# nquach/TEE_optical_flow

Measured on AMD Instinct MI355X. Metric: frame-pairs/sec @512x512 DualTVL1, higher is better.
Workload: dtype f32

## Files before the change

tee_optical_flow_amd/csrc/teeflow_dbg.hip.h:

```cpp
namespace {
template <class T> struct DevBuf { T* p = nullptr; ~DevBuf() { if (p) (void)hipFree(p); } };
using DBuf = DevBuf<float>;

int dbg_up(tf_handle* h, DBuf& d, const float* src, const Geom& g)
{
    HIPC(h, hipMalloc(&d.p, (size_t)g.plane * sizeof(float)));
    HIPC(h, hipMemsetAsync(d.p, 0, (size_t)g.plane * sizeof(float), h->stream));
    if (src) HIPC(h, hipMemcpy2DAsync(d.p, (size_t)g.pitch * 4, src, (size_t)g.w * 4, (size_t)g.w * 4, g.h, hipMemcpyHostToDevice, h->stream));
    return TF_OK;
}
int dbg_down(tf_handle* h, float* dst, const float* d, const Geom& g)
{
    HIPC(h, hipMemcpy2DAsync(dst, (size_t)g.w * 4, d, (size_t)g.pitch * 4, (size_t)g.w * 4, g.h, hipMemcpyDeviceToHost, h->stream));
    HIPC(h, hipStreamSynchronize(h->stream));
    return TF_OK;
}

int dbg_up2(tf_handle* h, DBuf& fr, const float* I0, const float* I1, const Geom& g)
{
    HIPC(h, hipMalloc(&fr.p, 2 * (size_t)g.plane * sizeof(float)));
    HIPC(h, hipMemsetAsync(fr.p, 0, 2 * (size_t)g.plane * sizeof(float), h->stream));
    HIPC(h, hipMemcpy2DAsync(fr.p, (size_t)g.pitch * 4, I0, (size_t)g.w * 4, (size_t)g.w * 4, g.h, hipMemcpyHostToDevice, h->stream));
    HIPC(h, hipMemcpy2DAsync(fr.p + g.plane, (size_t)g.pitch * 4, I1, (size_t)g.w * 4, (size_t)g.w * 4, g.h, hipMemcpyHostToDevice, h->stream));
    return TF_OK;
// ... 204 lines not shown
    const Geom g = make_geom(w, hgt);
    DBuf a0, a1, b0, b1;
    int rc;
    if ((rc = dbg_up(h, a0, src, g)) || (rc = dbg_up(h, a1, nullptr, g)) || (rc = dbg_up(h, b0, src, g)) || (rc = dbg_up(h, b1, nullptr, g))) return rc;
    DevBuf<PairCtl> ctl;
    HIPC(h, hipMalloc(&ctl.p, sizeof(PairCtl)));
    HIPC(h, hipMemsetAsync(ctl.p, 0, sizeof(PairCtl), h->stream));
    MedArgs ma = {};
    ma.sb.u1[0] = a0.p; ma.sb.u1[1] = a1.p; ma.sb.u2[0] = b0.p; ma.sb.u2[1] = b1.p;
    ma.ctl = ctl.p; ma.err = nullptr; ma.errstride = 0; ma.it = 0; ma.thr_q = 0; ma.utog = 0; ma.g = g;
    ma.total = 1; ma.step = iter_step(h, false, h->P.inner_iterations);
    const dim3 gm((g.w + 63) / 64, (g.h + 15) / 16, 2);
    if (ksize == 5) hipLaunchKernelGGL(k_median<5>, gm, dim3(256), 0, h->stream, ma);
    else hipLaunchKernelGGL(k_median<3>, gm, dim3(256), 0, h->stream, ma);
    hipError_t e = hipStreamSynchronize(h->stream);
    if (e != hipSuccess) return fail(h, TF_ERR_HIP, "k_median: %s", hipGetErrorString(e));
    return dbg_down(h, dst, a1.p, g);
}

TF_API int tf_dbg_iterate(tf_handle* h, const float* I1wx, const float* I1wy, const float* rho_c,
                          float* u1, float* u2, float* p11, float* p12, float* p21, float* p22,
                          int w, int hgt, int nsteps, int p_is_zero, unsigned long long* err_q)
{
    if (!h || !I1wx || !I1wy || !rho_c || !u1 || !u2 || !p11 || !p12 || !p21 || !p22 || w < 1 || hgt < 1 || nsteps < 0)
        return TF_ERR_INVALID_ARG;
    HIPC(h, hipSetDevice(h->dev));
    const Geom g = make_geom(w, hgt);
    DBuf cx, cy, cr, s[12];
    int rc;
    if ((rc = dbg_up(h, cx, I1wx, g)) || (rc = dbg_up(h, cy, I1wy, g)) || (rc = dbg_up(h, cr, rho_c, g))) return rc;
    float* hostp[6] = {u1, u2, p11, p12, p21, p22};
    for (int k = 0; k < 6; ++k) {
        if ((rc = dbg_up(h, s[2 * k], hostp[k], g)) || (rc = dbg_up(h, s[2 * k + 1], nullptr, g))) return rc;
    }
    DevBuf<PairCtl> ctl; DevBuf<u64> errs;
    HIPC(h, hipMalloc(&ctl.p, sizeof(PairCtl)));
    HIPC(h, hipMemsetAsync(ctl.p, 0, sizeof(PairCtl), h->stream));
    HIPC(h, hipMalloc(&errs.p, (size_t)(nsteps + 1) * sizeof(u64)));
    HIPC(h, hipMemsetAsync(errs.p, 0, (size_t)(nsteps + 1) * sizeof(u64), h->stream));
    Iter2Args A = {};
    IterArgs& ia = A.a;
    ia.wx = cx.p; ia.wy = cy.p; ia.rho = cr.p;
    for (int k = 0; k < 2; ++k) {
        ia.sb.u1[k] = s[0 + k].p; ia.sb.u2[k] = s[2 + k].p; ia.sb.p11[k] = s[4 + k].p;
        ia.sb.p12[k] = s[6 + k].p; ia.sb.p21[k] = s[8 + k].p; ia.sb.p22[k] = s[10 + k].p;
    }
    ia.ctl = ctl.p; ia.err = errs.p; ia.errstride = nsteps + 1; ia.thr_q = -1.0; ia.g = g; ia.host_slot = nullptr; ia.B = 1;
    ia.l_t = (float)(h->P.lambda * h->P.theta); ia.theta = (float)h->P.theta; ia.taut = (float)(h->P.tau / h->P.theta);
    const int step = iter_step(h, false, nsteps);
    A.total = nsteps;
    int launches = 0;
    for (int it = 0; it < nsteps; it += step, ++launches) {
        ia.it = it; ia.utog = ia.ptog = launches; ia.pzero = (p_is_zero && it == 0) ? 1 : 0;
        launch_iter(h, A, step, 1, h->stream);
    }
    hipError_t e = hipStreamSynchronize(h->stream);
    if (e == hipSuccess && err_q && nsteps > 0) {
        e = hipMemcpyAsync(err_q, errs.p, (size_t)nsteps * sizeof(u64), hipMemcpyDeviceToHost, h->stream);
        if (e == hipSuccess) e = hipStreamSynchronize(h->stream);
    }
    if (e != hipSuccess) return fail(h, TF_ERR_HIP, "k_iter: %s", hipGetErrorString(e));
    const int cur = launches & 1;
    for (int k = 0; k < 6; ++k)
        if ((rc = dbg_down(h, hostp[k], s[2 * k + cur].p, g))) return rc;
    return TF_OK;
}
```

tee_optical_flow_amd/csrc/teeflow_tvl1_host.hip.h:

```cpp
namespace {
int validate_params(Engine* h, const tf_params& p)
{
    if (p.algo != TF_ALGO_TVL1) return fail(h, TF_ERR_UNSUPPORTED, "algo %d not implemented (only TF_ALGO_TVL1)", p.algo);
    if (p.nscales < 1 || p.nscales > MAXLEV) return fail(h, TF_ERR_INVALID_ARG, "nscales must be in [1,%d], got %d", MAXLEV, p.nscales);
    if (p.warps < 1) return fail(h, TF_ERR_INVALID_ARG, "warps must be >= 1, got %d", p.warps);
    if (p.inner_iterations < 1 || p.outer_iterations < 1)
        return fail(h, TF_ERR_INVALID_ARG, "inner/outer iterations must be >= 1, got %d/%d", p.inner_iterations, p.outer_iterations);
    if ((long long)p.inner_iterations * p.outer_iterations > 100000)
        return fail(h, TF_ERR_INVALID_ARG, "inner*outer iterations too large");
    if (p.median_filtering != 1 && p.median_filtering != 3 && p.median_filtering != 5)
        return fail(h, TF_ERR_UNSUPPORTED, "medianFiltering must be 1, 3 or 5 (cv::medianBlur on CV_32F), got %d", p.median_filtering);
    if (p.gamma != 0.0) return fail(h, TF_ERR_UNSUPPORTED, "gamma != 0 (illumination term u3) is not implemented");
    if (p.variant != TF_VARIANT_CPU && p.variant != TF_VARIANT_CUDA) return fail(h, TF_ERR_INVALID_ARG, "variant must be TF_VARIANT_CPU or TF_VARIANT_CUDA, got %d", p.variant);
    if (p.variant == TF_VARIANT_CUDA && (p.inner_iterations * p.outer_iterations) % 2 != 0)
        return fail(h, TF_ERR_UNSUPPORTED, "TF_VARIANT_CUDA needs an even iteration count (inner*outer), got %d", p.inner_iterations * p.outer_iterations);
    if (p.use_initial_flow && p.variant == TF_VARIANT_CUDA)
        return fail(h, TF_ERR_UNSUPPORTED, "useInitialFlow is not implemented for TF_VARIANT_CUDA (nothing checks that form bit for bit)");
    if (!(p.scale_step > 0.0 && p.scale_step < 1.0)) return fail(h, TF_ERR_INVALID_ARG, "scaleStep must be in (0,1), got %g", p.scale_step);
    if (p.scale_step == 0.5) return fail(h, TF_ERR_UNSUPPORTED, "scaleStep == 0.5 makes cv::resize take its INTER_AREA fast path for the pyramid, which is not implemented");
    if (!(p.theta > 0.0) || !(p.tau > 0.0) || !(p.lambda > 0.0) || !(p.epsilon >= 0.0))
        return fail(h, TF_ERR_INVALID_ARG, "tau, lambda, theta must be > 0 and epsilon >= 0");
    return TF_OK;
}

// ... 32 lines not shown
    HIPC(e, hipStreamSynchronize(e->stream));
    release(); release_staging(e);
    nlev = compute_levels(P, H_, W_, lv);
    const size_t ncap = (size_t)want_cap, fcap = 2 * ncap;
    for (int l = 0; l < nlev; ++l) HIPC(e, hipMalloc(&pyr[l], fcap * lv[l].plane * sizeof(float)));
    if (P.variant == TF_VARIANT_CUDA)
        for (int l = 0; l < nlev; ++l) {
            HIPC(e, hipMalloc(&gxl[l], fcap * lv[l].plane * sizeof(float)));
            HIPC(e, hipMalloc(&gyl[l], fcap * lv[l].plane * sizeof(float)));
        }
    variant = P.variant;
    const size_t pl = (size_t)lv[0].plane * ncap * sizeof(float);
    HIPC(e, hipMalloc(&cwx, pl)); HIPC(e, hipMalloc(&cwy, pl)); HIPC(e, hipMalloc(&crho, pl));
    for (int k = 0; k < 2; ++k) {
        HIPC(e, hipMalloc(&sb.u1[k], pl)); HIPC(e, hipMalloc(&sb.u2[k], pl));
        HIPC(e, hipMalloc(&sb.p11[k], pl)); HIPC(e, hipMalloc(&sb.p12[k], pl));
        HIPC(e, hipMalloc(&sb.p21[k], pl)); HIPC(e, hipMalloc(&sb.p22[k], pl));
    }
    HIPC(e, hipMalloc(&ctl, ncap * sizeof(PairCtl)));
    errstride = total;
    HIPC(e, hipMalloc(&errs, ncap * (size_t)errstride * sizeof(u64)));
    iters_cap = ncap * (size_t)nlev * (size_t)P.warps * 2;
    HIPC(e, hipMalloc(&iters_dev, iters_cap * sizeof(int)));
    H = H_; W = W_; cap = want_cap;
    scale_step = P.scale_step; nscales = P.nscales;
    return TF_OK;
}

inline dim3 grid64x4(const Geom& g, int z) { return dim3((g.w + 63) / 64, (g.h + 3) / 4, z); }

bool rows_ok(const Engine* h, const Geom& g, int B)
{
    return h->iter_variant >= 1 && g.w <= h->max_strip_width && (long long)g.h * B >= h->min_rows_work;
}

int iter_step(const Engine* h, bool cuda_variant, int inner)
{
    return (cuda_variant || (h->iter_variant >= 2 && inner % 2 == 0)) ? 2 : 1;
}

void strip_shape(const Engine* h, const Geom& g, int B, int* R, int* QX, int* RY, int* threads)
{
    const int qx = (g.w + 3) / 4;
    int ry = 256 / qx;
    if (ry < 1) ry = 1;
    *QX = qx; *RY = ry;
    *threads = qx * ry <= 256 ? 256 : (qx * ry + 63) / 64 * 64;
    long long n = (long long)g.h * B / ((long long)h->strip_blocks * ry);
    if (n < 2) n = 2;
    if (n > 16) n = 16;
    *R = ry * (int)n;
}

void launch_iter(Engine* h, const Iter2Args& A, int step, int B, hipStream_t s)
{
    const Geom& g = A.a.g;
    if (!rows_ok(h, g, B)) {
        if (step == 2) hipLaunchKernelGGL(k_iter2_tile, dim3((g.w + T2_OW - 1) / T2_OW, (g.h + T2_OH - 1) / T2_OH, B), dim3(256), 0, s, A);
        else hipLaunchKernelGGL(k_iter, dim3((g.w + IT_OW - 1) / IT_OW, (g.h + IT_OH - 1) / IT_OH, B), dim3(256), 0, s, A.a);
        return;
    }
    int R, QX, RY, threads;
    strip_shape(h, g, B, &R, &QX, &RY, &threads);
    const int LW = QX * 4 + 4;
    if (step == 1) {
        const size_t shmem1 = (size_t)(32 + 8 * RY * LW + 2 * RY * QX) * sizeof(float);
        hipLaunchKernelGGL(k_iter_rows, dim3((g.h + R - 1) / R, 1, B), dim3(threads), shmem1, s, A.a, R, QX, RY);
        return;
    }
    const size_t shmem = (size_t)(32 + 8 * RY * LW + 2 * (RY + 1) * LW + 2 * RY * QX) * sizeof(float);
    if (B <= 1024) {
        auto f = h->tv.slots_cache.find(shmem * 1024 + (size_t)threads / 64);
        if (f == h->tv.slots_cache.end()) {
            int per_cu = 0;
            (void)hipOccupancyMaxActiveBlocksPerMultiprocessor(&per_cu, k_iter2_rows, threads, shmem);
            if (per_cu < 1) per_cu = 1;
            f = h->tv.slots_cache.emplace(shmem * 1024 + (size_t)threads / 64, per_cu * h->num_cus).first;
        }
        int slots = f->second;
        if (h->slots_pct > 0 && h->slots_pct < 100) slots = slots * h->slots_pct / 100;
        int items = 1;
        for (int n = 1; n <= B; ++n) {
            int r, sn;
            strip_rule(n, g.h, RY, slots, &r, &sn);
            if (n * sn > items) items = n * sn;
        }
        hipLaunchKernelGGL(k_iter2_rows, dim3(items, 1, 1), dim3(threads), shmem, s, A, 0, QX, RY, slots);
        return;
    }
    hipLaunchKernelGGL(k_iter2_rows, dim3((g.h + R - 1) / R, 1, B), dim3(threads), shmem, s, A, R, QX, RY, 0);
}

inline int warp_margin_class(int m) { return m <= 0 ? 0 : (m <= 4 ? 4 : (m <= 8 ? 8 : 16)); }
void launch_warp(Engine* h, const WarpArgs& wa, int B, hipStream_t s, const float* gx = nullptr, const float* gy = nullptr)
{
    const Geom& g = wa.g;
    if (h->P.variant == TF_VARIANT_CUDA) {
        WarpCudaArgs ca; ca.w = wa; ca.gx = gx; ca.gy = gy;
        hipLaunchKernelGGL(k_warp_cuda, dim3((g.w + 63) / 64, (g.h + 3) / 4, B), dim3(256), 0, s, ca);
        return;
    }
    const int M = warp_margin_class(h->warp_margin);
    const dim3 grid((g.w + WL_TW - 1) / WL_TW, (g.h + WL_TH - 1) / WL_TH, B);
    const size_t shm = (size_t)(128 + (WL_TW + 2 * (M + 4)) * (WL_TH + 2 * M + 7)) * sizeof(float);
    switch (M) {
        case 4: hipLaunchKernelGGL(k_warp_lds<4>, grid, dim3(256), shm, s, wa); break;
        case 8: hipLaunchKernelGGL(k_warp_lds<8>, grid, dim3(256), shm, s, wa); break;
        case 16: hipLaunchKernelGGL(k_warp_lds<16>, grid, dim3(256), shm, s, wa); break;
        default: hipLaunchKernelGGL(k_warp, dim3((g.w + 63) / 64, (g.h + 3) / 4, B), dim3(256), 0, s, wa); break;
    }
}

int read_reports(Engine* h, hipStream_t s, unsigned q, unsigned* checked, bool* stop)
{
    while (*checked <= q) {
        int v = h->tv.slots_host[*checked % SLOT_RING];
        if (v < 0) {
            if (q - *checked < (unsigned)DEFAULT_LAG) break;
            const double t0 = now_ms();
            while ((v = h->tv.slots_host[*checked % SLOT_RING]) < 0) {
                if (now_ms() - t0 > 20000.0) return fail(h, TF_ERR_HIP, "tvl1_iter launch %u never reported (GPU hang?)", *checked);
                if (hipStreamQuery(s) == hipSuccess && h->tv.slots_host[*checked % SLOT_RING] < 0)
                    return fail(h, TF_ERR_HIP, "stream drained but launch %u did not report", *checked);
            }
        }
        ++*checked;
        if (v == 0) { *stop = true; break; }
    }
    return TF_OK;
}

int run_stage(Engine* h, int l, int wi, int B, int off0, int off1)
{
    const tf_params& P = h->P;
    const Geom g = h->tv.lv[l];
    const int inner = P.inner_iterations, total = P.inner_iterations * P.outer_iterations;
    const float thr_f = (float)(P.epsilon * P.epsilon * (double)(g.w * g.h));
    const double thr_q = (double)thr_f * 1073741824.0;
    const double thr_d = P.epsilon * P.epsilon * (double)(g.w * g.h);
    hipStream_t s = h->stream;

    WarpArgs wa;
    wa.pyr = h->tv.pyr[l]; wa.off0 = off0; wa.off1 = off1; wa.sb = h->tv.sb; wa.ctl = h->tv.ctl; wa.tab = h->tv.tab;
    wa.wx = h->tv.cwx; wa.wy = h->tv.cwy; wa.rho = h->tv.crho; wa.g = g;
    int rc = profiled(h, s, -4, 0, 0, [&] { launch_warp(h, wa, B, s, h->tv.gxl[l], h->tv.gyl[l]); });
    if (rc) return rc;
    HIPC(h, hipMemsetAsync(h->tv.errs, 0, (size_t)B * h->tv.errstride * sizeof(u64), s));

    Iter2Args A;
    IterArgs& ia = A.a;
    ia.wx = h->tv.cwx; ia.wy = h->tv.cwy; ia.rho = h->tv.crho; ia.sb = h->tv.sb; ia.ctl = h->tv.ctl; ia.err = h->tv.errs;
    ia.errstride = h->tv.errstride; ia.thr_q = thr_q; ia.g = g;
    ia.l_t = (float)(P.lambda * P.theta); ia.theta = (float)P.theta; ia.taut = (float)(P.tau / P.theta);
    ia.variant = P.variant; ia.thr_d = thr_d;
    const bool cuda_variant = P.variant == TF_VARIANT_CUDA;
    const bool median = P.median_filtering > 1 && !cuda_variant;
    MedArgs ma;
    ma.sb = h->tv.sb; ma.ctl = h->tv.ctl; ma.err = h->tv.errs; ma.errstride = h->tv.errstride; ma.thr_q = thr_q; ma.g = g;

    const dim3 gm((g.w + 63) / 64, (g.h + 15) / 16, 2 * B);
    ia.B = B;
    const int step = iter_step(h, cuda_variant, inner);
    ma.total = A.total = total; ma.step = step;
    A.utog_prev = A.ptog_prev = A.pzero_prev = 0;
    int utog = 0, ptog = 0;
    bool stop = false;
    unsigned checked = h->tv.launch_seq;
    for (int it = 0; it < total + step - 1 && !stop; it += step) {
        if (it < total && it % inner == 0 && median) {
            ma.it = it; ma.utog = utog;
            rc = profiled(h, s, -5, 0, 0, [&] {
                if (P.median_filtering == 5) hipLaunchKernelGGL(k_median<5>, gm, dim3(256), 0, s, ma);
                else hipLaunchKernelGGL(k_median<3>, gm, dim3(256), 0, s, ma);
            });
            if (rc) return rc;
            ++utog;
        }
        const unsigned q = h->tv.launch_seq++;
        h->tv.slots_host[q % SLOT_RING] = -1;
        ia.host_slot = h->tv.slots_dev + q % SLOT_RING;
        ia.it = it; ia.utog = utog; ia.ptog = ptog; ia.pzero = (wi == 0 && it == 0) ? 1 : 0;
        rc = profiled(h, s, l, wi, it, [&] { launch_iter(h, A, step, B, s); });
        if (rc) return rc;
        ++h->tally.iter_launches;
        A.utog_prev = utog; A.ptog_prev = ptog; A.pzero_prev = ia.pzero;
        ++utog; ++ptog;
        rc = read_reports(h, s, q, &checked, &stop);
        if (rc) return rc;
    }
    hipLaunchKernelGGL(k_stage_end, dim3((B + 255) / 256), dim3(256), 0, s, h->tv.errs, h->tv.errstride, h->tv.ctl, h->tv.iters_dev, B,
                       total, inner, median ? 1 : 0, thr_q, l, wi, h->tv.nlev, P.warps, P.variant, thr_d, step);
    return TF_OK;
}

int solve_resident(Engine* h, const uint8_t* dframes, bool f32, int F, int B, int off0, int off1, float scale, void* dflow, bool out_f16,
                   const float* dinit = nullptr)
{
    const tf_params& P = h->P;
    hipStream_t s = h->stream;
    const Geom g0 = h->tv.lv[0];
    if (f32) hipLaunchKernelGGL(k_f32_to_level0, dim3((g0.w + 255) / 256, g0.h, F), dim3(256), 0, s, (const float*)dframes, h->tv.pyr[0], g0, 1);
    else hipLaunchKernelGGL(k_u8_to_f32, dim3((g0.w + 255) / 256, g0.h, F), dim3(256), 0, s, dframes, h->tv.pyr[0], g0);
    for (int l = 1; l < h->tv.nlev; ++l) {
        const double sc = 1.0 / P.scale_step;
        hipLaunchKernelGGL(k_pyr_down, grid64x4(h->tv.lv[l], F), dim3(256), 0, s, h->tv.pyr[l - 1], h->tv.lv[l - 1], h->tv.pyr[l], h->tv.lv[l], sc, sc,
                           P.variant == TF_VARIANT_CUDA ? 1 : 0);
    }
    if (P.variant == TF_VARIANT_CUDA)
        for (int l = 0; l < h->tv.nlev; ++l)
            hipLaunchKernelGGL(k_grad, grid64x4(h->tv.lv[l], F), dim3(256), 0, s, h->tv.pyr[l], h->tv.gxl[l], h->tv.gyl[l], h->tv.lv[l]);
    const int L = h->tv.nlev - 1;
    hipLaunchKernelGGL(k_ctl_set, dim3((B + 255) / 256), dim3(256), 0, s, h->tv.ctl, B, 0);
    const auto seed_step = [&](int l) {
        if (l == 0) hipLaunchKernelGGL(k_init_split, grid64x4(g0, B), dim3(256), 0, s, dinit, h->tv.sb, L & 1, g0);
        else hipLaunchKernelGGL(k_init_down, grid64x4(h->tv.lv[l], B), dim3(256), 0, s, h->tv.sb, (L - l + 1) & 1, h->tv.lv[l - 1], h->tv.lv[l],
                                1.0 / P.scale_step, (float)P.scale_step);
    };
    if (dinit) for (int l = 0; l < L; ++l) seed_step(l);
    HIPC(h, hipMemset2DAsync(h->tv.sb.u1[0], (size_t)h->tv.lv[L].splane * sizeof(float), 0, (size_t)h->tv.lv[L].plane * sizeof(float), B, s));
    HIPC(h, hipMemset2DAsync(h->tv.sb.u2[0], (size_t)h->tv.lv[L].splane * sizeof(float), 0, (size_t)h->tv.lv[L].plane * sizeof(float), B, s));
    if (dinit) seed_step(L);
    for (int l = L; l >= 0; --l) {
        for (int wi = 0; wi < P.warps; ++wi) {
            int rc = run_stage(h, l, wi, B, off0, off1);
            if (rc) return rc;
        }
        if (l == 0) break;
        const Geom gs = h->tv.lv[l], gd = h->tv.lv[l - 1];
        const double sx = 1.0 / ((double)gd.w / gs.w), sy = 1.0 / ((double)gd.h / gs.h);
        hipLaunchKernelGGL(k_flow_up, grid64x4(gd, B), dim3(256), 0, s, h->tv.sb, h->tv.ctl, gs, gd, sx, sy, (float)(1 / P.scale_step),
                           P.variant == TF_VARIANT_CUDA ? 1 : 0);
        hipLaunchKernelGGL(k_ctl_set, dim3((B + 255) / 256), dim3(256), 0, s, h->tv.ctl, B, 1);
    }
    if (out_f16) hipLaunchKernelGGL(k_output<uint16_t>, out_grid<uint16_t>(g0, B), dim3(256), 0, s, h->tv.sb, h->tv.ctl, g0, scale, (uint16_t*)dflow);
    else hipLaunchKernelGGL(k_output<float>, out_grid<float>(g0, B), dim3(256), 0, s, h->tv.sb, h->tv.ctl, g0, scale, (float*)dflow);
    HIPC(h, hipGetLastError());
// ... 27 lines not shown
```

tee_optical_flow_amd/csrc/teeflow_tvl1_iter.hip.h:

```cpp
#pragma once

__device__ __forceinline__ bool pair_active(const u64* errb, int it, double thr_q)
{
    if (it == 0) return true;
    return (double)errb[it - 1] > thr_q;
}

#define IT_TW 64
#define IT_TH 16
#define IT_OW 60
#define IT_OH 15

struct IterArgs {
    const float *wx, *wy, *rho;
    StateBufs sb;
    const PairCtl* ctl;
    u64* err; int errstride; int it; double thr_q;
    int utog, ptog, pzero;
    Geom g;
    float l_t, theta, taut;
    int* host_slot;
    int B;
    int variant;
    double thr_d;
// ... 459 lines not shown
            const double err = (double)e[n] * 0x1p-30;
            prev = err;
            if (!(err > thr)) { if (n_it) *n_it = n + 1; return M_EXIT; }
        } else prev -= thr;
    }
    if (n_it) *n_it = total;
    return it < total ? M_NORMAL : M_EXIT;
}

__device__ __forceinline__ int pair_mode(const u64* e, int it, int total, double thr_q, int variant, double thr_d)
{
    return variant ? pair_mode_cuda(e, it, total, thr_d, nullptr) : pair_mode2(e, it, total, thr_q);
}

TF_HD inline void strip_rule_min(int n, int H, int minrows, int slots, int* R, int* S)
{
    if (n < 1) n = 1;
    if (minrows < 1) minrows = 1;
    const int k = (n + slots - 1) / slots;
    int s = (int)(((long long)k * slots) / n);
    const int smax = H / minrows > 0 ? H / minrows : 1;
    if (s > smax) s = smax;
    if (s < 1) s = 1;
    int r = (H + s - 1) / s;
    *R = r;
    *S = (H + r - 1) / r;
}
TF_HD inline void strip_rule(int n, int H, int RY, int slots, int* R, int* S)
{
    strip_rule_min(n, H, 4 * RY, slots, R, S);
}

struct Iter2Args {
    IterArgs a;
    int utog_prev, ptog_prev, pzero_prev;
    int total;
};

__device__ __forceinline__ void publish_active_count2(const Iter2Args& A)
{
    const IterArgs& a = A.a;
    if (a.host_slot && blockIdx.x == 0 && blockIdx.y == 0 && blockIdx.z == 0 && threadIdx.x < 64) {
        int c = 0;
        for (int b2 = threadIdx.x; b2 < a.B; b2 += 64)
            c += pair_mode(a.err + (size_t)b2 * a.errstride, a.it, A.total, a.thr_q, a.variant, a.thr_d) != M_EXIT ? 1 : 0;
#pragma unroll
        for (int off = 32; off > 0; off >>= 1) c += __shfl_down(c, off, 64);
        if (threadIdx.x == 0) __hip_atomic_store(a.host_slot, c, __ATOMIC_RELAXED, __HIP_MEMORY_SCOPE_SYSTEM);
    }
}


struct Iter2Blk {
    int b, strip, R, QX, RY;
    bool replay, pzero;
    int uc, pc;
    int it;
    u64* errb;
    int W, H, pitch;
    long long splane;
};

__device__ __forceinline__ void iter2_rows_body(const IterArgs& a, const Iter2Blk& k, float* smem);

__global__ __launch_bounds__(512) void k_iter2_rows(Iter2Args A, int R, int QX, int RY, int slots)
{
    extern __shared__ __attribute__((aligned(16))) float smem[];
    const IterArgs& a = A.a;
    u64* sred = reinterpret_cast<u64*>(smem);

    publish_active_count2(A);
    int b = blockIdx.z, strip = blockIdx.x;
    if (slots > 0) {
        const int nchunk = (a.B + 63) >> 6, nw = (int)(blockDim.x >> 6), wv = (int)(threadIdx.x >> 6), ln = (int)(threadIdx.x & 63);
        for (int c = wv; c < nchunk; c += nw) {
            const int pb = c * 64 + ln;
            const bool on = pb < a.B && pair_mode(a.err + (size_t)pb * a.errstride, a.it, A.total, a.thr_q, a.variant, a.thr_d) != M_EXIT;
            const u64 m = __ballot(on);
            if (ln == 0) sred[c] = m;
        }
        __syncthreads();
        int nact = 0;
        for (int c = 0; c < nchunk; ++c) nact += __popcll(sred[c]);
        int S;
        strip_rule(nact, a.g.h, RY, slots, &R, &S);
        const int item = blockIdx.x;
        if (item >= nact * S) return;
        int k = item / S;
        strip = item - k * S;
        int c = 0;
        u64 m = sred[0];
        while (k >= __popcll(m)) { k -= __popcll(m); m = sred[++c]; }
        for (; k > 0; --k) m &= m - 1;
        b = c * 64 + (__ffsll((long long)m) - 1);
        __syncthreads();
    }
    u64* errb = a.err + (size_t)b * a.errstride;
    const int mode = pair_mode(errb, a.it, A.total, a.thr_q, a.variant, a.thr_d);
    if (mode == M_EXIT) return;
    const bool replay = mode == M_REPLAY;
    const PairCtl c = a.ctl[b];
    const int utog = replay ? A.utog_prev : a.utog, ptog = replay ? A.ptog_prev : a.ptog;
    Iter2Blk blk;
    blk.b = b; blk.strip = strip; blk.R = R; blk.QX = QX; blk.RY = RY; blk.replay = replay;
    blk.pzero = (replay ? A.pzero_prev : a.pzero) != 0;
    blk.uc = (c.ubase ^ utog) & 1; blk.pc = (c.pbase ^ ptog) & 1;
    blk.it = a.it; blk.errb = errb;
    blk.W = a.g.w; blk.H = a.g.h; blk.pitch = a.g.pitch; blk.splane = a.g.splane;
    iter2_rows_body(a, blk, smem);
}

__device__ __forceinline__ void iter2_rows_body(const IterArgs& a, const Iter2Blk& k, float* smem)
{
    const int b = k.b, strip = k.strip, R = k.R, QX = k.QX, RY = k.RY, uc = k.uc, pc = k.pc;
    const bool replay = k.replay, pzero = k.pzero;
    u64* errb = k.errb;
    const int LW = QX * 4 + 4;
    u64* sred = reinterpret_cast<u64*>(smem);
    float* U1a = smem + 32;
    float* U1b = U1a + 2 * RY * LW;
    float* U2a = U1b + 2 * RY * LW;
    float* U2b = U2a + 2 * RY * LW;
    float* B12 = U2b + 2 * RY * LW;
    float* B22 = B12 + (RY + 1) * LW;
    float* B11w = B22 + (RY + 1) * LW;
    float* B21w = B11w + RY * QX;
    const int tid = threadIdx.x;
    const int ty = tid / QX, tx = tid - ty * QX;
    const bool lane_on = ty < RY;
    const int W = k.W, H = k.H, pitch = k.pitch;
    const int x = tx * 4;
    const int y0 = strip * R;
    const int ngroups = (R + 3 + RY - 1) / RY;
    const size_t po = (size_t)b * (size_t)k.splane;
    const int RB = RY + 1;

    const float* __restrict__ gu1 = a.sb.u1[uc] + po;
    const float* __restrict__ gu2 = a.sb.u2[uc] + po;
    const float* __restrict__ g11 = a.sb.p11[pc] + po;
    const float* __restrict__ g12 = a.sb.p12[pc] + po;
    const float* __restrict__ g21 = a.sb.p21[pc] + po;
    const float* __restrict__ g22 = a.sb.p22[pc] + po;
    const float* __restrict__ gwx = a.wx + po;
    const float* __restrict__ gwy = a.wy + po;
    const float* __restrict__ grh = a.rho + po;
    float* __restrict__ ou1 = a.sb.u1[uc ^ 1] + po;
    float* __restrict__ ou2 = a.sb.u2[uc ^ 1] + po;
    float* __restrict__ o11 = a.sb.p11[pc ^ 1] + po;
    float* __restrict__ o12 = a.sb.p12[pc ^ 1] + po;
    float* __restrict__ o21 = a.sb.p21[pc ^ 1] + po;
    float* __restrict__ o22 = a.sb.p22[pc ^ 1] + po;

    const int yu1_lo = y0 - 1, yu1_hi = y0 + R + 1, yp1_hi = y0 + R, yout_hi = y0 + R - 1;

    float s1_u1[4], s1_u2[4], s1_wx[4], s1_wy[4], s1_r[4], s1_11[4], s1_12[4], s1_21[4], s1_22[4];
    float s2_u1[4], s2_u2[4], s2_11[4], s2_12[4], s2_21[4], s2_22[4];
#pragma unroll
    for (int i = 0; i < 4; ++i) {
        s1_u1[i] = s1_u2[i] = s1_wx[i] = s1_wy[i] = s1_r[i] = s1_11[i] = s1_12[i] = s1_21[i] = s1_22[i] = 0.f;
        s2_u1[i] = s2_u2[i] = s2_11[i] = s2_12[i] = s2_21[i] = s2_22[i] = 0.f;
    }
    bool s1_valid = false, s2_valid = false;
    unsigned inw[5];
#pragma unroll
    for (int j = 0; j < 5; ++j) inw[j] = opaque_u(x + j < W ? ~0u : 0u);
    int ring = ty + 1;
    u64 qA = 0, qB = 0;
    double accA = 0.0, accB = 0.0;

    for (int s = 0; s < ngroups + 2; ++s) {
        const int r1 = s * RY + ty;
        const int y = y0 - 1 + r1;
        const bool v1 = lane_on && s < ngroups && y >= 0 && y < H && y >= yu1_lo && y <= yu1_hi;
        const size_t row = (size_t)y * pitch + x;
        float4 u1q, u2q, wxq, wyq, rq, a11, a12, a21, a22;
        u1q = u2q = wxq = wyq = rq = a11 = a12 = a21 = a22 = make_float4(0, 0, 0, 0);
        if (v1) {
            u1q = ld4(gu1 + row); u2q = ld4(gu2 + row);
            wxq = ld4(gwx + row); wyq = ld4(gwy + row); rq = ld4(grh + row);
            if (!pzero) { a11 = ld4(g11 + row); a12 = ld4(g12 + row); a21 = ld4(g21 + row); a22 = ld4(g22 + row); }
        }
        float n_u1[4] = {0, 0, 0, 0}, n_u2[4] = {0, 0, 0, 0};
        float c11[4], c12[4], c21[4], c22[4], wxv[4], wyv[4], rv[4];
        UNPACK4(c11, a11) UNPACK4(c12, a12) UNPACK4(c21, a21) UNPACK4(c22, a22) UNPACK4(wxv, wxq) UNPACK4(wyv, wyq) UNPACK4(rv, rq)
        if (v1) {
            float4 up12 = make_float4(0, 0, 0, 0), up22 = up12;
            if (y > 0 && !pzero) { up12 = ld4(g12 + row - pitch); up22 = ld4(g22 + row - pitch); }
            float l11 = 0.f, l21 = 0.f;
            if (tx > 0 && !pzero) { l11 = g11[row - 1]; l21 = g21[row - 1]; }
            QuadU qu;
            UNPACK4(qu.u1k, u1q) UNPACK4(qu.u2k, u2q) UNPACK4(qu.wx, wxq) UNPACK4(qu.wy, wyq) UNPACK4(qu.r, rq)
            UNPACK4(qu.p11, a11) UNPACK4(qu.p12, a12) UNPACK4(qu.p21, a21) UNPACK4(qu.p22, a22)
            UNPACK4(qu.p12u, up12) UNPACK4(qu.p22u, up22)
            qu.l11 = l11; qu.l21 = l21;
            const bool isout = y >= y0 && y <= yout_hi;
            tv_u_quad_pk(a.l_t, a.theta, qu, y == 0, x == 0, n_u1, n_u2);
            const unsigned mrow = opaque_u(!replay && isout ? ~0u : 0u);
            const unsigned keep[4] = {inw[0] & mrow, inw[1] & mrow, inw[2] & mrow, inw[3] & mrow};
            accA += tv_err_quad_pk(n_u1, qu.u1k, n_u2, qu.u2k, keep);
            st4(U1a + ((s & 1) * RY + ty) * LW + x, PACK4(n_u1));
            st4(U1b + ((s & 1) * RY + ty) * LW + x, PACK4(n_u2));
        }
        __syncthreads();
        const int yb = y - RY;
        const bool v2 = s1_valid && yb <= yp1_hi;
        float p1_11[4] = {0, 0, 0, 0}, p1_12[4] = {0, 0, 0, 0}, p1_21[4] = {0, 0, 0, 0}, p1_22[4] = {0, 0, 0, 0};
        if (v2) {
            const int bp = (s - 1) & 1;
            const bool lastrow = yb >= H - 1;
            float4 dn1 = make_float4(0, 0, 0, 0), dn2 = dn1;
            if (!lastrow) {
                const float* d1 = ty < RY - 1 ? U1a + (bp * RY + ty + 1) * LW + x : U1a + ((s & 1) * RY) * LW + x;
                const float* d2 = ty < RY - 1 ? U1b + (bp * RY + ty + 1) * LW + x : U1b + ((s & 1) * RY) * LW + x;
                dn1 = ld4(d1); dn2 = ld4(d2);
            }
            float rr1 = 0.f, rr2 = 0.f;
            if (x + 4 < W) { rr1 = U1a[(bp * RY + ty) * LW + x + 4]; rr2 = U1b[(bp * RY + ty) * LW + x + 4]; }
            const unsigned mnl = opaque_u(lastrow ? 0u : ~0u);
            float dv1[4], dv2[4], u1x[4], u1y[4], u2x[4], u2y[4];
            UNPACK4(dv1, dn1) UNPACK4(dv2, dn2)
            {
                const float4 o1 = ld4(U1a + (bp * RY + ty) * LW + x), o2 = ld4(U1b + (bp * RY + ty) * LW + x);
                UNPACK4(s1_u1, o1) UNPACK4(s1_u2, o2)
            }
#pragma unroll
            for (int i = 0; i < 4; ++i) {
                const float e1 = i < 3 ? s1_u1[i + 1] : rr1, e2 = i < 3 ? s1_u2[i + 1] : rr2;
                u1x[i] = mask_f(e1 - s1_u1[i], inw[i + 1]);
                u2x[i] = mask_f(e2 - s1_u2[i], inw[i + 1]);
                u1y[i] = mask_f(dv1[i] - s1_u1[i], mnl);
                u2y[i] = mask_f(dv2[i] - s1_u2[i], mnl);
            }
            tv_p_quad_pk(a.taut, u1x, u1y, u2x, u2y, s1_11, s1_12, s1_21, s1_22, p1_11, p1_12, p1_21, p1_22);
            if (replay) {
                if (yb >= y0 && yb <= yout_hi) {
                    const size_t prow = (size_t)yb * pitch + x;
                    st4(ou1 + prow, PACK4(s1_u1)); st4(ou2 + prow, PACK4(s1_u2));
                    st4(o11 + prow, PACK4(p1_11)); st4(o12 + prow, PACK4(p1_12));
                    st4(o21 + prow, PACK4(p1_21)); st4(o22 + prow, PACK4(p1_22));
                }
            } else {
                st4(B12 + ring * LW + x, PACK4(p1_12));
                st4(B22 + ring * LW + x, PACK4(p1_22));
                B11w[ty * QX + tx] = p1_11[3];
                B21w[ty * QX + tx] = p1_21[3];
            }
        }
        bool v2u = false;
        float m_u1[4] = {0, 0, 0, 0}, m_u2[4] = {0, 0, 0, 0};
        if (!replay) {
            __syncthreads();
            v2u = v2 && yb >= y0;
            if (v2u) {
                float4 up12 = make_float4(0, 0, 0, 0), up22 = up12;
                if (yb > 0) {
                    const int ri = ring > 0 ? ring - 1 : RB - 1;
                    up12 = ld4(B12 + ri * LW + x); up22 = ld4(B22 + ri * LW + x);
                }
                float l11 = 0.f, l21 = 0.f;
                if (tx > 0) { l11 = B11w[ty * QX + tx - 1]; l21 = B21w[ty * QX + tx - 1]; }
                QuadU qu;
#pragma unroll
                for (int i = 0; i < 4; ++i) {
                    qu.u1k[i] = s1_u1[i]; qu.u2k[i] = s1_u2[i]; qu.wx[i] = s1_wx[i]; qu.wy[i] = s1_wy[i]; qu.r[i] = s1_r[i];
                    qu.p11[i] = p1_11[i]; qu.p12[i] = p1_12[i]; qu.p21[i] = p1_21[i]; qu.p22[i] = p1_22[i];
                }
                UNPACK4(qu.p12u, up12) UNPACK4(qu.p22u, up22)
                qu.l11 = l11; qu.l21 = l21;
                const bool isout = yb <= yout_hi;
                tv_u_quad_pk(a.l_t, a.theta, qu, yb == 0, x == 0, m_u1, m_u2);
                const unsigned mrow = opaque_u(isout ? ~0u : 0u);
                const unsigned keep[4] = {inw[0] & mrow, inw[1] & mrow, inw[2] & mrow, inw[3] & mrow};
                accB += tv_err_quad_pk(m_u1, s1_u1, m_u2, s1_u2, keep);
                st4(U2a + (((s - 1) & 1) * RY + ty) * LW + x, PACK4(m_u1));
                st4(U2b + (((s - 1) & 1) * RY + ty) * LW + x, PACK4(m_u2));
            }
            __syncthreads();
            const int yc = y - 2 * RY;
            if (s2_valid && yc <= yout_hi) {
                const int bq = s & 1;
                const bool lastrow = yc >= H - 1;
                float4 dn1 = make_float4(0, 0, 0, 0), dn2 = dn1;
                if (!lastrow) {
                    const float* d1 = ty < RY - 1 ? U2a + (bq * RY + ty + 1) * LW + x : U2a + ((bq ^ 1) * RY) * LW + x;
                    const float* d2 = ty < RY - 1 ? U2b + (bq * RY + ty + 1) * LW + x : U2b + ((bq ^ 1) * RY) * LW + x;
                    dn1 = ld4(d1); dn2 = ld4(d2);
                }
                float rr1 = 0.f, rr2 = 0.f;
                if (x + 4 < W) { rr1 = U2a[(bq * RY + ty) * LW + x + 4]; rr2 = U2b[(bq * RY + ty) * LW + x + 4]; }
                const unsigned mnl = opaque_u(lastrow ? 0u : ~0u);
                float dv1[4], dv2[4], r11[4], r12[4], r21[4], r22[4], u1x[4], u1y[4], u2x[4], u2y[4];
                UNPACK4(dv1, dn1) UNPACK4(dv2, dn2)
                {
                    const float4 o1 = ld4(U2a + (bq * RY + ty) * LW + x), o2 = ld4(U2b + (bq * RY + ty) * LW + x);
                    UNPACK4(s2_u1, o1) UNPACK4(s2_u2, o2)
                }
#pragma unroll
                for (int i = 0; i < 4; ++i) {
                    const float e1 = i < 3 ? s2_u1[i + 1] : rr1, e2 = i < 3 ? s2_u2[i + 1] : rr2;
                    u1x[i] = mask_f(e1 - s2_u1[i], inw[i + 1]);
                    u2x[i] = mask_f(e2 - s2_u2[i], inw[i + 1]);
                    u1y[i] = mask_f(dv1[i] - s2_u1[i], mnl);
                    u2y[i] = mask_f(dv2[i] - s2_u2[i], mnl);
                }
                tv_p_quad_pk(a.taut, u1x, u1y, u2x, u2y, s2_11, s2_12, s2_21, s2_22, r11, r12, r21, r22);
                const size_t prow = (size_t)yc * pitch + x;
                st4(ou1 + prow, PACK4(s2_u1)); st4(ou2 + prow, PACK4(s2_u2));
                st4(o11 + prow, PACK4(r11)); st4(o12 + prow, PACK4(r12));
                st4(o21 + prow, PACK4(r21)); st4(o22 + prow, PACK4(r22));
            }
        }
        else __syncthreads();
        s2_valid = v2u;
#pragma unroll
        for (int i = 0; i < 4; ++i) {
            s2_11[i] = p1_11[i]; s2_12[i] = p1_12[i]; s2_21[i] = p1_21[i]; s2_22[i] = p1_22[i];
            s1_wx[i] = wxv[i]; s1_wy[i] = wyv[i]; s1_r[i] = rv[i];
            s1_11[i] = c11[i]; s1_12[i] = c12[i]; s1_21[i] = c21[i]; s1_22[i] = c22[i];
        }
        s1_valid = v1;
        ring += RY; ring = ring >= RB ? ring - RB : ring;
        if ((s & 255) == 255) { qA += (u64)accA; qB += (u64)accB; accA = accB = 0.0; }
    }
    if (!replay) {
        qA += (u64)accA; qB += (u64)accB;
#pragma unroll
        for (int off = 32; off > 0; off >>= 1) { qA += __shfl_down(qA, off, 64); qB += __shfl_down(qB, off, 64); }
        __syncthreads();
        if ((tid & 63) == 0) { sred[tid >> 6] = qA; sred[8 + (tid >> 6)] = qB; }
        __syncthreads();
        if (tid == 0) {
            u64 ta = 0, tb = 0;
            for (int w = 0; w < (int)(blockDim.x >> 6); ++w) { ta += sred[w]; tb += sred[8 + w]; }
            atomicAdd(&errb[k.it], ta);
            atomicAdd(&errb[k.it + 1], tb);
        }
    }
}

#define T2_OW 52
#define T2_OH 13

__global__ __launch_bounds__(256) void k_iter2_tile(Iter2Args A)
{
    constexpr int LW = 68;
    __shared__ __attribute__((aligned(16))) float sA[16][LW], sB[16][LW];
    __shared__ __attribute__((aligned(16))) float s12[16][LW], s22[16][LW];
    __shared__ float s11w[16][16], s21w[16][16];
    __shared__ u64 sred[8];
    const IterArgs& a = A.a;
    publish_active_count2(A);
    const int b = blockIdx.z;
    u64* errb = a.err + (size_t)b * a.errstride;
    const int mode = pair_mode(errb, a.it, A.total, a.thr_q, a.variant, a.thr_d);
    if (mode == M_EXIT) return;
    const bool replay = mode == M_REPLAY;
    const PairCtl c = a.ctl[b];
    const int utog = replay ? A.utog_prev : a.utog, ptog = replay ? A.ptog_prev : a.ptog;
    const bool pzero = (replay ? A.pzero_prev : a.pzero) != 0;
    const int uc = (c.ubase ^ utog) & 1, pc = (c.pbase ^ ptog) & 1;
    const int tx = threadIdx.x & 15, ty = threadIdx.x >> 4;
    const int W = a.g.w, H = a.g.h, pitch = a.g.pitch;
    const int x = (int)blockIdx.x * T2_OW - 4 + tx * 4, y = (int)blockIdx.y * T2_OH - 1 + ty;
    const bool inr = x >= 0 && x < W && y >= 0 && y < H;
    const bool outq = inr && tx >= 1 && tx <= 13 && ty >= 1 && ty <= 13;
    const size_t po = (size_t)b * a.g.splane;
    const size_t row = po + (size_t)(inr ? y : 0) * pitch + (inr ? x : 0);

    unsigned inw[5];
#pragma unroll
    for (int j = 0; j < 5; ++j) inw[j] = opaque_u(x + j < W ? ~0u : 0u);
    const unsigned mnl = opaque_u(y >= H - 1 ? 0u : ~0u);
    const unsigned mout = opaque_u(outq ? ~0u : 0u);
    const unsigned keep[4] = {inw[0] & mout, inw[1] & mout, inw[2] & mout, inw[3] & mout};
// ... 132 lines not shown
```

Measured before the change: 2889.

## Linearize k_iter2_rows work over quads so every thread stays busy each step

The fused two-iteration strip kernel no longer maps one row per thread-row with idle lanes when the row width does not divide the block. Instead each step assigns T consecutive quads in raster order, with each thread advancing its own (y,x) position and using circular LDS rings sized by thread count. This removes idle lanes (ty >= RY) and shrinks or regularizes the LDS footprint. In exchange it adds per-thread index bookkeeping, column-mask recomputation, and an occupancy check that fails the launch if fewer than three 256-thread blocks fit per CU.

After: 2921 (median of 6 runs). 1.01x the previous value.

```diff
diff --git a/tee_optical_flow_amd/csrc/teeflow_dbg.hip.h b/tee_optical_flow_amd/csrc/teeflow_dbg.hip.h
--- a/tee_optical_flow_amd/csrc/teeflow_dbg.hip.h
+++ b/tee_optical_flow_amd/csrc/teeflow_dbg.hip.h
@@ -280,7 +280,8 @@
     int launches = 0;
     for (int it = 0; it < nsteps; it += step, ++launches) {
         ia.it = it; ia.utog = ia.ptog = launches; ia.pzero = (p_is_zero && it == 0) ? 1 : 0;
-        launch_iter(h, A, step, 1, h->stream);
+        const int lrc = launch_iter(h, A, step, 1, h->stream);
+        if (lrc) return lrc;
     }
     hipError_t e = hipStreamSynchronize(h->stream);
     if (e == hipSuccess && err_q && nsteps > 0) {
diff --git a/tee_optical_flow_amd/csrc/teeflow_tvl1_host.hip.h b/tee_optical_flow_amd/csrc/teeflow_tvl1_host.hip.h
--- a/tee_optical_flow_amd/csrc/teeflow_tvl1_host.hip.h
+++ b/tee_optical_flow_amd/csrc/teeflow_tvl1_host.hip.h
@@ -108,28 +108,31 @@
     *R = ry * (int)n;
 }
 
-void launch_iter(Engine* h, const Iter2Args& A, int step, int B, hipStream_t s)
+int launch_iter(Engine* h, const Iter2Args& A, int step, int B, hipStream_t s)
 {
     const Geom& g = A.a.g;
     if (!rows_ok(h, g, B)) {
         if (step == 2) hipLaunchKernelGGL(k_iter2_tile, dim3((g.w + T2_OW - 1) / T2_OW, (g.h + T2_OH - 1) / T2_OH, B), dim3(256), 0, s, A);
         else hipLaunchKernelGGL(k_iter, dim3((g.w + IT_OW - 1) / IT_OW, (g.h + IT_OH - 1) / IT_OH, B), dim3(256), 0, s, A.a);
-        return;
+        return TF_OK;
     }
     int R, QX, RY, threads;
     strip_shape(h, g, B, &R, &QX, &RY, &threads);
-    const int LW = QX * 4 + 4;
     if (step == 1) {
+        const int LW = QX * 4 + 4;
         const size_t shmem1 = (size_t)(32 + 8 * RY * LW + 2 * RY * QX) * sizeof(float);
         hipLaunchKernelGGL(k_iter_rows, dim3((g.h + R - 1) / R, 1, B), dim3(threads), shmem1, s, A.a, R, QX, RY);
-        return;
-    }
-    const size_t shmem = (size_t)(32 + 8 * RY * LW + 2 * (RY + 1) * LW + 2 * RY * QX) * sizeof(float);
+        return TF_OK;
+    }
+    if (QX > threads) return fail(h, TF_ERR_HIP, "k_iter2_rows: %d quads per row do not fit a block of %d threads", QX, threads);
+    const size_t shmem = (size_t)(32 + 4 * 8 * threads + 2 * 4 * (threads + QX) + 2 * (threads + QX)) * sizeof(float);
     if (B <= 1024) {
         auto f = h->tv.slots_cache.find(shmem * 1024 + (size_t)threads / 64);
         if (f == h->tv.slots_cache.end()) {
             int per_cu = 0;
             (void)hipOccupancyMaxActiveBlocksPerMultiprocessor(&per_cu, k_iter2_rows, threads, shmem);
+            if (threads == 256 && per_cu < 3)
+                return fail(h, TF_ERR_HIP, "k_iter2_rows: %d blocks per CU with %zu B of LDS, 3 expected", per_cu, shmem);
             if (per_cu < 1) per_cu = 1;
             f = h->tv.slots_cache.emplace(shmem * 1024 + (size_t)threads / 64, per_cu * h->num_cus).first;
         }
@@ -142,9 +145,10 @@
             if (n * sn > items) items = n * sn;
         }
         hipLaunchKernelGGL(k_iter2_rows, dim3(items, 1, 1), dim3(threads), shmem, s, A, 0, QX, RY, slots);
-        return;
+        return TF_OK;
     }
     hipLaunchKernelGGL(k_iter2_rows, dim3((g.h + R - 1) / R, 1, B), dim3(threads), shmem, s, A, R, QX, RY, 0);
+    return TF_OK;
 }
 
 inline int warp_margin_class(int m) { return m <= 0 ? 0 : (m <= 4 ? 4 : (m <= 8 ? 8 : 16)); }
@@ -236,8 +240,9 @@
         h->tv.slots_host[q % SLOT_RING] = -1;
         ia.host_slot = h->tv.slots_dev + q % SLOT_RING;
         ia.it = it; ia.utog = utog; ia.ptog = ptog; ia.pzero = (wi == 0 && it == 0) ? 1 : 0;
-        rc = profiled(h, s, l, wi, it, [&] { launch_iter(h, A, step, B, s); });
-        if (rc) return rc;
+        int lrc = TF_OK;
+        rc = profiled(h, s, l, wi, it, [&] { lrc = launch_iter(h, A, step, B, s); });
+        if (rc || lrc) return rc ? rc : lrc;
         ++h->tally.iter_launches;
         A.utog_prev = utog; A.ptog_prev = ptog; A.pzero_prev = ia.pzero;
         ++utog; ++ptog;
diff --git a/tee_optical_flow_amd/csrc/teeflow_tvl1_iter.hip.h b/tee_optical_flow_amd/csrc/teeflow_tvl1_iter.hip.h
--- a/tee_optical_flow_amd/csrc/teeflow_tvl1_iter.hip.h
+++ b/tee_optical_flow_amd/csrc/teeflow_tvl1_iter.hip.h
@@ -535,7 +535,7 @@
 
 
 struct Iter2Blk {
-    int b, strip, R, QX, RY;
+    int b, strip, R, QX;
     bool replay, pzero;
     int uc, pc;
     int it;
@@ -585,7 +585,7 @@
     const PairCtl c = a.ctl[b];
     const int utog = replay ? A.utog_prev : a.utog, ptog = replay ? A.ptog_prev : a.ptog;
     Iter2Blk blk;
-    blk.b = b; blk.strip = strip; blk.R = R; blk.QX = QX; blk.RY = RY; blk.replay = replay;
+    blk.b = b; blk.strip = strip; blk.R = R; blk.QX = QX; blk.replay = replay;
     blk.pzero = (replay ? A.pzero_prev : a.pzero) != 0;
     blk.uc = (c.ubase ^ utog) & 1; blk.pc = (c.pbase ^ ptog) & 1;
     blk.it = a.it; blk.errb = errb;
@@ -595,28 +595,27 @@
 
 __device__ __forceinline__ void iter2_rows_body(const IterArgs& a, const Iter2Blk& k, float* smem)
 {
-    const int b = k.b, strip = k.strip, R = k.R, QX = k.QX, RY = k.RY, uc = k.uc, pc = k.pc;
+    const int b = k.b, strip = k.strip, R = k.R, QX = k.QX, uc = k.uc, pc = k.pc;
     const bool replay = k.replay, pzero = k.pzero;
     u64* errb = k.errb;
-    const int LW = QX * 4 + 4;
+    const int T = (int)blockDim.x;
+    const int NU = 8 * T, NB = T + QX;
     u64* sred = reinterpret_cast<u64*>(smem);
     float* U1a = smem + 32;
-    float* U1b = U1a + 2 * RY * LW;
-    float* U2a = U1b + 2 * RY * LW;
-    float* U2b = U2a + 2 * RY * LW;
-    float* B12 = U2b + 2 * RY * LW;
-    float* B22 = B12 + (RY + 1) * LW;
-    float* B11w = B22 + (RY + 1) * LW;
-    float* B21w = B11w + RY * QX;
+    float* U1b = U1a + NU;
+    float* U2a = U1b + NU;
+    float* U2b = U2a + NU;
+    float* B12 = U2b + NU;
+    float* B22 = B12 + 4 * NB;
+    float* B11w = B22 + 4 * NB;
+    float* B21w = B11w + NB;
     const int tid = threadIdx.x;
-    const int ty = tid / QX, tx = tid - ty * QX;
-    const bool lane_on = ty < RY;
     const int W = k.W, H = k.H, pitch = k.pitch;
-    const int x = tx * 4;
     const int y0 = strip * R;
-    const int ngroups = (R + 3 + RY - 1) / RY;
+    const int nsteps = ((R + 3) * QX + T - 1) / T;
+    const int dy = T / QX, dx = (T - dy * QX) * 4;
+    const int xend = QX * 4, xlast = xend - 4;
     const size_t po = (size_t)b * (size_t)k.splane;
-    const int RB = RY + 1;
 
     const float* __restrict__ gu1 = a.sb.u1[uc] + po;
     const float* __restrict__ gu2 = a.sb.u2[uc] + po;
@@ -634,7 +633,7 @@
     float* __restrict__ o21 = a.sb.p21[pc ^ 1] + po;
     float* __restrict__ o22 = a.sb.p22[pc ^ 1] + po;
 
-    const int yu1_lo = y0 - 1, yu1_hi = y0 + R + 1, yp1_hi = y0 + R, yout_hi = y0 + R - 1;
+    const int yu1_hi = y0 + R + 1, yp1_hi = y0 + R, yout_hi = y0 + R - 1;
 
     float s1_u1[4], s1_u2[4], s1_wx[4], s1_wy[4], s1_r[4], s1_11[4], s1_12[4], s1_21[4], s1_22[4];
     float s2_u1[4], s2_u2[4], s2_11[4], s2_12[4], s2_21[4], s2_22[4];
@@ -644,17 +643,29 @@
         s2_u1[i] = s2_u2[i] = s2_11[i] = s2_12[i] = s2_21[i] = s2_22[i] = 0.f;
     }
     bool s1_valid = false, s2_valid = false;
-    unsigned inw[5];
-#pragma unroll
-    for (int j = 0; j < 5; ++j) inw[j] = opaque_u(x + j < W ? ~0u : 0u);
-    int ring = ty + 1;
+    unsigned wm[5];
+#pragma unroll
+    for (int j = 1; j < 5; ++j) wm[j] = xlast + j < W ? ~0u : 0u;
+    const auto col_masks = [&](int xq, unsigned* m) {
+        const bool last = xq == xlast;
+        m[0] = ~0u;
+#pragma unroll
+        for (int j = 1; j < 5; ++j) m[j] = opaque_u(last ? wm[j] : ~0u);
+    };
+    const int ty0 = tid / QX;
+    int y1 = y0 - 1 + ty0, x1 = (tid - ty0 * QX) * 4, y2 = 0, x2 = 0, y3 = 0, x3 = 0;
+    int bpos = tid + QX;
+    int rtA = tid * 4 + 4, dnA = tid * 4 + xend;
+    int rtX = 4 * T + tid * 4 + 4, dnX = 4 * T + tid * 4 + xend;
+    rtX = (rtX == NU ? 0 : rtX) ^ rtA; dnX = (dnX >= NU ? dnX - NU : dnX) ^ dnA;
     u64 qA = 0, qB = 0;
     double accA = 0.0, accB = 0.0;
 
-    for (int s = 0; s < ngroups + 2; ++s) {
-        const int r1 = s * RY + ty;
-        const int y = y0 - 1 + r1;
-        const bool v1 = lane_on && s < ngroups && y >= 0 && y < H && y >= yu1_lo && y <= yu1_hi;
+    for (int s = 0; s < nsteps + 2; ++s) {
+        const int own1 = (s & 1) * 4 * T + tid * 4;
+        const int own2 = 4 * T - (s & 1) * 4 * T + tid * 4;
+        const int y = y1, x = x1;
+        const bool v1 = y >= 0 && y < H && y <= yu1_hi;
         const size_t row = (size_t)y * pitch + x;
         float4 u1q, u2q, wxq, wyq, rq, a11, a12, a21, a22;
         u1q = u2q = wxq = wyq = rq = a11 = a12 = a21 = a22 = make_float4(0, 0, 0, 0);
@@ -670,7 +681,7 @@
             float4 up12 = make_float4(0, 0, 0, 0), up22 = up12;
             if (y > 0 && !pzero) { up12 = ld4(g12 + row - pitch); up22 = ld4(g22 + row - pitch); }
             float l11 = 0.f, l21 = 0.f;
-            if (tx > 0 && !pzero) { l11 = g11[row - 1]; l21 = g21[row - 1]; }
+            if (x > 0 && !pzero) { l11 = g11[row - 1]; l21 = g21[row - 1]; }
             QuadU qu;
             UNPACK4(qu.u1k, u1q) UNPACK4(qu.u2k, u2q) UNPACK4(qu.wx, wxq) UNPACK4(qu.wy, wyq) UNPACK4(qu.r, rq)
             UNPACK4(qu.p11, a11) UNPACK4(qu.p12, a12) UNPACK4(qu.p21, a21) UNPACK4(qu.p22, a22)
@@ -678,32 +689,32 @@
             qu.l11 = l11; qu.l21 = l21;
             const bool isout = y >= y0 && y <= yout_hi;
             tv_u_quad_pk(a.l_t, a.theta, qu, y == 0, x == 0, n_u1, n_u2);
+            unsigned inw[5];
+            col_masks(x, inw);
             const unsigned mrow = opaque_u(!replay && isout ? ~0u : 0u);
             const unsigned keep[4] = {inw[0] & mrow, inw[1] & mrow, inw[2] & mrow, inw[3] & mrow};
             accA += tv_err_quad_pk(n_u1, qu.u1k, n_u2, qu.u2k, keep);
-            st4(U1a + ((s & 1) * RY + ty) * LW + x, PACK4(n_u1));
-            st4(U1b + ((s & 1) * RY + ty) * LW + x, PACK4(n_u2));
+            st4(U1a + own1, PACK4(n_u1));
+            st4(U1b + own1, PACK4(n_u2));
         }
         __syncthreads();
-        const int yb = y - RY;
+        const int yb = y2, xb = x2;
         const bool v2 = s1_valid && yb <= yp1_hi;
         float p1_11[4] = {0, 0, 0, 0}, p1_12[4] = {0, 0, 0, 0}, p1_21[4] = {0, 0, 0, 0}, p1_22[4] = {0, 0, 0, 0};
+        unsigned inw[5];
+        col_masks(xb, inw);
         if (v2) {
-            const int bp = (s - 1) & 1;
+            const int rt = rtA ^ rtX, dn = dnA ^ dnX;
             const bool lastrow = yb >= H - 1;
             float4 dn1 = make_float4(0, 0, 0, 0), dn2 = dn1;
-            if (!lastrow) {
-                const float* d1 = ty < RY - 1 ? U1a + (bp * RY + ty + 1) * LW + x : U1a + ((s & 1) * RY) * LW + x;
-                const float* d2 = ty < RY - 1 ? U1b + (bp * RY + ty + 1) * LW + x : U1b + ((s & 1) * RY) * LW + x;
-                dn1 = ld4(d1); dn2 = ld4(d2);
-            }
+            if (!lastrow) { dn1 = ld4(U1a + dn); dn2 = ld4(U1b + dn); }
             float rr1 = 0.f, rr2 = 0.f;
-            if (x + 4 < W) { rr1 = U1a[(bp * RY + ty) * LW + x + 4]; rr2 = U1b[(bp * RY + ty) * LW + x + 4]; }
+            if (xb != xlast) { rr1 = U1a[rt]; rr2 = U1b[rt]; }
             const unsigned mnl = opaque_u(lastrow ? 0u : ~0u);
             float dv1[4], dv2[4], u1x[4], u1y[4], u2x[4], u2y[4];
             UNPACK4(dv1, dn1) UNPACK4(dv2, dn2)
             {
-                const float4 o1 = ld4(U1a + (bp * RY + ty) * LW + x), o2 = ld4(U1b + (bp * RY + ty) * LW + x);
+                const float4 o1 = ld4(U1a + own2), o2 = ld4(U1b + own2);
                 UNPACK4(s1_u1, o1) UNPACK4(s1_u2, o2)
             }
 #pragma unroll
@@ -717,16 +728,16 @@
             tv_p_quad_pk(a.taut, u1x, u1y, u2x, u2y, s1_11, s1_12, s1_21, s1_22, p1_11, p1_12, p1_21, p1_22);
             if (replay) {
                 if (yb >= y0 && yb <= yout_hi) {
-                    const size_t prow = (size_t)yb * pitch + x;
+                    const size_t prow = (size_t)yb * pitch + xb;
                     st4(ou1 + prow, PACK4(s1_u1)); st4(ou2 + prow, PACK4(s1_u2));
                     st4(o11 + prow, PACK4(p1_11)); st4(o12 + prow, PACK4(p1_12));
                     st4(o21 + prow, PACK4(p1_21)); st4(o22 + prow, PACK4(p1_22));
                 }
             } else {
-                st4(B12 + ring * LW + x, PACK4(p1_12));
-                st4(B22 + ring * LW + x, PACK4(p1_22));
-                B11w[ty * QX + tx] = p1_11[3];
-                B21w[ty * QX + tx] = p1_21[3];
+                st4(B12 + bpos * 4, PACK4(p1_12));
+                st4(B22 + bpos * 4, PACK4(p1_22));
+                B11w[bpos] = p1_11[3];
+                B21w[bpos] = p1_21[3];
             }
         }
         bool v2u = false;
@@ -737,11 +748,14 @@
             if (v2u) {
                 float4 up12 = make_float4(0, 0, 0, 0), up22 = up12;
                 if (yb > 0) {
-                    const int ri = ring > 0 ? ring - 1 : RB - 1;
-                    up12 = ld4(B12 + ri * LW + x); up22 = ld4(B22 + ri * LW + x);
+                    const int up = bpos >= QX ? bpos - QX : bpos - QX + NB;
+                    up12 = ld4(B12 + up * 4); up22 = ld4(B22 + up * 4);
                 }
                 float l11 = 0.f, l21 = 0.f;
-                if (tx > 0) { l11 = B11w[ty * QX + tx - 1]; l21 = B21w[ty * QX + tx - 1]; }
+                if (xb > 0) {
+                    const int lf = bpos > 0 ? bpos - 1 : NB - 1;
+                    l11 = B11w[lf]; l21 = B21w[lf];
+                }
                 QuadU qu;
 #pragma unroll
                 for (int i = 0; i < 4; ++i) {
@@ -751,43 +765,41 @@
                 UNPACK4(qu.p12u, up12) UNPACK4(qu.p22u, up22)
                 qu.l11 = l11; qu.l21 = l21;
                 const bool isout = yb <= yout_hi;
-                tv_u_quad_pk(a.l_t, a.theta, qu, yb == 0, x == 0, m_u1, m_u2);
+                tv_u_quad_pk(a.l_t, a.theta, qu, yb == 0, xb == 0, m_u1, m_u2);
                 const unsigned mrow = opaque_u(isout ? ~0u : 0u);
                 const unsigned keep[4] = {inw[0] & mrow, inw[1] & mrow, inw[2] & mrow, inw[3] & mrow};
                 accB += tv_err_quad_pk(m_u1, s1_u1, m_u2, s1_u2, keep);
-                st4(U2a + (((s - 1) & 1) * RY + ty) * LW + x, PACK4(m_u1));
-                st4(U2b + (((s - 1) & 1) * RY + ty) * LW + x, PACK4(m_u2));
+                st4(U2a + own2, PACK4(m_u1));
+                st4(U2b + own2, PACK4(m_u2));
             }
             __syncthreads();
-            const int yc = y - 2 * RY;
+            const int yc = y3, xc = x3;
             if (s2_valid && yc <= yout_hi) {
-                const int bq = s & 1;
+                const int rt = rtA, dn = dnA;
                 const bool lastrow = yc >= H - 1;
                 float4 dn1 = make_float4(0, 0, 0, 0), dn2 = dn1;
-                if (!lastrow) {
-                    const float* d1 = ty < RY - 1 ? U2a + (bq * RY + ty + 1) * LW + x : U2a + ((bq ^ 1) * RY) * LW + x;
-                    const float* d2 = ty < RY - 1 ? U2b + (bq * RY + ty + 1) * LW + x : U2b + ((bq ^ 1) * RY) * LW + x;
-                    dn1 = ld4(d1); dn2 = ld4(d2);
-                }
+                if (!lastrow) { dn1 = ld4(U2a + dn); dn2 = ld4(U2b + dn); }
                 float rr1 = 0.f, rr2 = 0.f;
-                if (x + 4 < W) { rr1 = U2a[(bq * RY + ty) * LW + x + 4]; rr2 = U2b[(bq * RY + ty) * LW + x + 4]; }
+                if (xc != xlast) { rr1 = U2a[rt]; rr2 = U2b[rt]; }
                 const unsigned mnl = opaque_u(lastrow ? 0u : ~0u);
+                unsigned inc[5];
+                col_masks(xc, inc);
                 float dv1[4], dv2[4], r11[4], r12[4], r21[4], r22[4], u1x[4], u1y[4], u2x[4], u2y[4];
                 UNPACK4(dv1, dn1) UNPACK4(dv2, dn2)
                 {
-                    const float4 o1 = ld4(U2a + (bq * RY + ty) * LW + x), o2 = ld4(U2b + (bq * RY + ty) * LW + x);
+                    const float4 o1 = ld4(U2a + own1), o2 = ld4(U2b + own1);
                     UNPACK4(s2_u1, o1) UNPACK4(s2_u2, o2)
                 }
 #pragma unroll
                 for (int i = 0; i < 4; ++i) {
                     const float e1 = i < 3 ? s2_u1[i + 1] : rr1, e2 = i < 3 ? s2_u2[i + 1] : rr2;
-                    u1x[i] = mask_f(e1 - s2_u1[i], inw[i + 1]);
-                    u2x[i] = mask_f(e2 - s2_u2[i], inw[i + 1]);
+                    u1x[i] = mask_f(e1 - s2_u1[i], inc[i + 1]);
+                    u2x[i] = mask_f(e2 - s2_u2[i], inc[i + 1]);
                     u1y[i] = mask_f(dv1[i] - s2_u1[i], mnl);
                     u2y[i] = mask_f(dv2[i] - s2_u2[i], mnl);
                 }
                 tv_p_quad_pk(a.taut, u1x, u1y, u2x, u2y, s2_11, s2_12, s2_21, s2_22, r11, r12, r21, r22);
-                const size_t prow = (size_t)yc * pitch + x;
+                const size_t prow = (size_t)yc * pitch + xc;
                 st4(ou1 + prow, PACK4(s2_u1)); st4(ou2 + prow, PACK4(s2_u2));
                 st4(o11 + prow, PACK4(r11)); st4(o12 + prow, PACK4(r12));
                 st4(o21 + prow, PACK4(r21)); st4(o22 + prow, PACK4(r22));
@@ -802,7 +814,11 @@
             s1_11[i] = c11[i]; s1_12[i] = c12[i]; s1_21[i] = c21[i]; s1_22[i] = c22[i];
         }
         s1_valid = v1;
-        ring += RY; ring = ring >= RB ? ring - RB : ring;
+        y3 = y2; x3 = x2; y2 = y1; x2 = x1;
+        y1 += dy; x1 += dx;
+        if (x1 >= xend) { x1 -= xend; ++y1; }
+        bpos += T; bpos = bpos >= NB ? bpos - NB : bpos;
+        rtA ^= rtX; dnA ^= dnX;
         if ((s & 255) == 255) { qA += (u64)accA; qB += (u64)accB; accA = accB = 0.0; }
     }
     if (!replay) {
```
